# ericyinyzy/VQAttack

Measured on AMD Instinct MI355X. Metric: adversarial_vqa_examples_per_sec, higher is better.
Workload: dtype f32; 1 GPU; vlmo_base VQAttack image PGD (BASELINE configs[1]): batch 64 per GPU, 40 PGD steps, 384x384 images, questions of 6..14 real tokens ([CLS] + n words + [SEP], n ~ U{4..12} seeded) padded to 40 (the all-padding columns are not run through the encoder), eps 0.125 step 0.01 L-inf clip [-1,1], random start, sanity_checks on, black-box scoring + ASR gather; batch_per_gpu=64, pgd_steps=40, image_size=384, text_len=40, substitutable_words=0

## Files before the change

### include/vqattack_hip.h

```cpp
#ifndef VQATTACK_HIP_H
#define VQATTACK_HIP_H

#include <stddef.h>
#include <stdint.h>

#ifdef __cplusplus
extern "C" {
#endif

typedef void* vqa_stream_t;

#define VQA_OK 0
#define VQA_ERR_NULL (-1)
#define VQA_ERR_SHAPE (-2)
#define VQA_ERR_ALIGN (-3)

#define VQA_CLIP 1u
#define VQA_CHECK_RANGE 2u
#define VQA_FLAG_RANGE 1
#define VQA_FLAG_BAD_LABEL 2
#define VQA_FLAG_DEGENERATE 4

int vqa_abi_version(void);
const char* vqa_error_string(int code);
// ... 64 lines not shown
int vqa_neg_cos_max_layers(void);
int vqa_neg_cos_rows_multi(const float* const* a, const float* const* b, float* const* ga, int n_layers,
                           float* partial, const uint8_t* row_mask, long mask_period, long rows0, long rows1, int D,
                           long a_stride0, long a_stride1, long b_stride0, long b_stride1, long g_stride0,
                           long g_stride1, float gscale, float cos_eps, float* loss_out, int accumulate,
                           vqa_stream_t stream);

int vqa_sum_partials(const float* partial, int count, float* dst, int accumulate, float scale,
                     vqa_stream_t stream);

int vqa_ce_max_label_sets(void);
long vqa_ce_scratch_floats(int K, long groups);
int vqa_ce_rows(const float* logits, long row_stride, const int64_t* labels, int K, long rows, int V,
                long ignore_index, long rows_per_group, float* scratch, float* grad, float* row_loss, float gscale,
                float* loss_out, int accumulate, int* flag, unsigned char* row_state, vqa_stream_t stream);

int vqa_gather_rows(const float* src, const int64_t* idx, float* dst, int B, int L, int K, int D,
                    vqa_stream_t stream);

int vqa_cand_dir_sim(const float* word, const float* pos, const float* type, const float* gamma,
                     const float* beta, float ln_eps, const float* e_ori, const float* grad,
                     const int32_t* cand, float* out, int n_cand, int L, int K, int D, vqa_stream_t stream);

int vqa_embed_tokens(const float* word, const float* pos, const float* type, const float* gamma, const float* beta,
                     float ln_eps, const int32_t* triples, int n, float* dst, int D, vqa_stream_t stream);

int vqa_greedy_accept(const int32_t* cand, const int32_t* order, const int32_t* seg, int B, int L,
                      const int64_t* ori_ids, int64_t* cur_ids, int32_t* new_id, int32_t* acc_rank, const float* table,
                      int V, int E, float threshold, vqa_stream_t stream);

int vqa_attn_fwd(const float* q, const float* k, const float* v, const float* bias, float* o, float* lse, float* scores,
                 int B, int H, int Sq, int Sk, const long* strides, const long* bias_strides, float scale,
                 const int* key_hole, int nsplit, float* split_ws, vqa_stream_t stream);
long vqa_attn_scores_floats(int B, int H, int Sq, int Sk);
long vqa_attn_split_ws_floats(int B, int H, int Sq, int Sk, int nsplit);

int vqa_attn_bwd(const float* q, const float* k, const float* v, const float* bias, const float* o, const float* go,
                 const float* lse, const float* scores, float* delta, float* dq, float* dk, float* dv, float* ds_ws, int B,
                 int H, int Sq, int Sk, const long* strides, const long* bias_strides, const long* grad_strides,
                 float scale, int nsplit, float* split_ws, vqa_stream_t stream);
long vqa_attn_bwd_ws_floats(int B, int H, int Sq, int Sk);

int vqa_resize_bicubic_h_u8(const uint8_t* src, int h, int w_in, int c, const int32_t* kk, const int32_t* bounds,
                            int ksize, int w_out, uint8_t* dst, vqa_stream_t stream);
int vqa_resize_bicubic_v_normalize(const uint8_t* src, int h_in, int w, int c, const int32_t* kk,
                                   const int32_t* bounds, int ksize, int h_out, float mean, float stdv, float* dst,
                                   vqa_stream_t stream);

int vqa_ln_fwd(const float* x, const float* r0, const float* r1, const float* rscale, float* x_out,
               const float* gamma0, const float* beta0, const float* gamma1, const float* beta1, float* y0, float* y1,
               float* mean, float* rstd, long rows, int D, long period, long split, float eps, vqa_stream_t stream);
int vqa_ln_bwd(const float* dy0, const float* dy1, const float* x, const float* mean, const float* rstd,
               const float* gamma0, const float* gamma1, const float* g_a, const float* g_inj, const float* rscale,
               float* dx, float* dr0, float* dr1, long rows, int D, long period, long split, vqa_stream_t stream);
int vqa_ln_bwd_post(const float* dy_a, const float* dy_b, const float* g_inj, const float* s, const float* rstd,
                    const float* gamma, float* ds, long rows, int D, vqa_stream_t stream);
int vqa_gelu_fwd(const float* h, float* a, size_t n, vqa_stream_t stream);
int vqa_gelu_bwd(const float* h, const float* da, float* dh, size_t n, vqa_stream_t stream);

size_t vqa_gemm_packed_bytes(int K, int N);
int vqa_gemm_pack_b(const float* w, long ldw, int trans, void* packed, int K, int N, vqa_stream_t stream);
int vqa_gemm_bf16x6(const float* A, long lda, const void* packed, const float* bias, float* C, long ldc, long M, int N,
                    int K, vqa_stream_t stream);

#define VQA_GEMM_TILE_256X128 0
#define VQA_GEMM_TILE_128X256 1
// ... 36 lines not shown
```

### vqattack_amd/_hip.py

```python
import ctypes
import os
import threading

import torch

_HERE = os.path.dirname(os.path.abspath(__file__))
LIB_PATH = os.path.join(_HERE, "lib", "libvqattack_hip.so")
TUNING_LIB_PATH = os.path.join(_HERE, "lib", "libvqattack_hip_tuning.so")

VQA_CLIP = 1
VQA_CHECK_RANGE = 2
VQA_FLAG_RANGE = 1
VQA_FLAG_BAD_LABEL = 2
VQA_FLAG_DEGENERATE = 4
ABI_VERSION = 4

_c_float_p = ctypes.c_void_p
_sz = ctypes.c_size_t
_f = ctypes.c_float
_i = ctypes.c_int
_u = ctypes.c_uint
_l = ctypes.c_long
_p = ctypes.c_void_p

SIGNATURES = {
    "vqa_abi_version": (_i, []),
    "vqa_error_string": (ctypes.c_char_p, [_i]),
    "vqa_linf_init": (_i, [_p, _p, _p, _sz, _f, _f, _f, _u, _p, _p]),
    "vqa_linf_fgm": (_i, [_p, _p, _p, _sz, _f, _f, _f, _u, _p, _p]),
    "vqa_linf_step": (_i, [_p, _p, _p, _p, _sz, _f, _f, _f, _f, _u, _p, _p]),
    "vqa_linf_project": (_i, [_p, _p, _p, _sz, _f, _f, _f, _u, _p]),
    "vqa_clip_eta_linf": (_i, [_p, _p, _sz, _f, _p]),
    "vqa_optimize_linear_linf": (_i, [_p, _p, _sz, _f, _p]),
    "vqa_zero_out_clipped_grads": (_i, [_p, _p, _p, _sz, _f, _f, _p]),
    "vqa_reduce_ws_bytes": (_sz, [_i, _sz]),
    "vqa_sumsq_per_sample": (_i, [_p, _p, _p, _i, _sz, _p, _p]),
    "vqa_absmax_ties_per_sample": (_i, [_p, _p, _p, _i, _sz, _p, _p]),
    "vqa_l2_fgm": (_i, [_p, _p, _p, _p, _i, _sz, _f, _f, _f, _u, _p, _p]),
    "vqa_l2_project": (_i, [_p, _p, _p, _p, _i, _sz, _f, _f, _f, _u, _p]),
    "vqa_l1_fgm": (_i, [_p, _p, _p, _p, _p, _i, _sz, _f, _f, _f, _u, _p, _p]),
    "vqa_scale_per_sample": (_i, [_p, _p, _p, _p, _i, _sz, _f, _i, _p, _p]),
    "vqa_sumabs_per_sample": (_i, [_p, _p, _i, _sz, _p, _p]),
    "vqa_momentum_accumulate": (_i, [_p, _p, _p, _i, _sz, _f, _p]),
    "vqa_linf_momentum_step": (_i, [_p, _p, _p, _p, _p, _p, _i, _sz, _f, _f, _f, _f, _f, _u, _p, _p]),
    "vqa_neg_cos_partials": (_i, []),
    "vqa_neg_cos_rows": (_i, [_p, _p, _p, _p, _p, _l, _l, _l, _i, _l, _l, _l, _l, _l, _l, _f, _f, _p, _i, _p]),
    "vqa_neg_cos_max_layers": (_i, []),
    "vqa_neg_cos_rows_multi": (_i, [_p, _p, _p, _i, _p, _p, _l, _l, _l, _i, _l, _l, _l, _l, _l, _l, _f, _f, _p, _i, _p]),
    "vqa_sum_partials": (_i, [_p, _i, _p, _i, _f, _p]),
    "vqa_ce_max_label_sets": (_i, []),
    "vqa_ce_scratch_floats": (_l, [_i, _l]),
    "vqa_ce_rows": (_i, [_p, _l, _p, _i, _l, _i, _l, _l, _p, _p, _p, _f, _p, _i, _p, _p, _p]),
    "vqa_gather_rows": (_i, [_p, _p, _p, _i, _i, _i, _i, _p]),
    "vqa_cand_dir_sim": (_i, [_p, _p, _p, _p, _p, _f, _p, _p, _p, _p, _i, _i, _i, _i, _p]),
    "vqa_embed_tokens": (_i, [_p, _p, _p, _p, _p, _f, _p, _i, _p, _i, _p]),
    "vqa_greedy_accept": (_i, [_p, _p, _p, _i, _i, _p, _p, _p, _p, _p, _i, _i, _f, _p]),
    "vqa_attn_fwd": (_i, [_p, _p, _p, _p, _p, _p, _p, _i, _i, _i, _i, _p, _p, _f, _p, _i, _p, _p]),
    "vqa_attn_split_ws_floats": (_l, [_i, _i, _i, _i, _i]),
    "vqa_attn_scores_floats": (_l, [_i, _i, _i, _i]),
    "vqa_attn_bwd": (_i, [_p, _p, _p, _p, _p, _p, _p, _p, _p, _p, _p, _p, _p, _i, _i, _i, _i, _p, _p, _p, _f, _i, _p, _p]),
    "vqa_attn_bwd_ws_floats": (_l, [_i, _i, _i, _i]),
    "vqa_ln_fwd": (_i, [_p] * 13 + [_l, _i, _l, _l, _f, _p]),
    "vqa_ln_bwd": (_i, [_p] * 13 + [_l, _i, _l, _l, _p]),
    "vqa_ln_bwd_post": (_i, [_p] * 7 + [_l, _i, _p]),
    "vqa_gelu_fwd": (_i, [_p, _p, _sz, _p]),
    "vqa_gelu_bwd": (_i, [_p, _p, _p, _sz, _p]),
    "vqa_resize_bicubic_h_u8": (_i, [_p, _i, _i, _i, _p, _p, _i, _i, _p, _p]),
    "vqa_resize_bicubic_v_normalize": (_i, [_p, _i, _i, _i, _p, _p, _i, _i, _f, _f, _p, _p]),
    "vqa_gemm_packed_bytes": (_sz, [_i, _i]),
    "vqa_gemm_pack_b": (_i, [_p, _l, _i, _p, _i, _i, _p]),
    "vqa_gemm_bf16x6": (_i, [_p, _l, _p, _p, _p, _l, _l, _i, _i, _p]),
    "vqa_gemm_bf16x6_tile": (_i, [_p, _l, _p, _p, _p, _l, _l, _i, _i, _i, _p]),
    "vqa_gemm_bf16x6_persistent": (_i, [_p, _l, _p, _p, _p, _l, _l, _i, _i, _i, _p]),
    "vqa_gemm_bf16x6_half": (_i, [_p, _l, _p, _p, _p, _l, _l, _i, _i, _p]),
    "vqa_gemm_bf16x6_tail": (_i, [_p, _l, _p, _p, _p, _l, _l, _i, _i, _i, _l, _p]),
    "vqa_gemm_small_ws_bytes": (_sz, [_l, _i, _i]),
    "vqa_gemm_bf16x6_small": (_i, [_p, _l, _p, _p, _p, _l, _l, _i, _i, _i, _p, _p]),
    "vqa_gemm_bf16x6_epi": (_i, [_p, _l, _p, _p, _p, _l, _l, _i, _i, _i, _i, _p, _l, _p]),
    "vqa_gemm_bf16x6_grouped": (_i, [_p, _p, _p, _p, _p, _p, _p, _p, _p, _i, _i, _i, _i, _p]),
    "vqa_gemm_lse_ws_floats": (_l, [_l, _i]),
    "vqa_gemm_bf16x6_lse": (_i, [_p, _l, _p, _p, _l, _i, _i, _i, _p, _l, _p, _p, _p, _p, _i, _p]),
}

_lib = None
_lock = threading.Lock()


class HipExtensionError(RuntimeError):
    pass

# ... 87 lines not shown
```

### vqattack_amd/attention.py

```python
import ctypes

import torch

from . import _hip
from ._hip import check, lib, ptr, stream_for

HEAD_DIM = 64


def _bshd(t, name):
    if not t.is_cuda or t.dtype != torch.float32 or t.dim() != 4 or t.shape[-1] != HEAD_DIM:
        raise _hip.HipExtensionError("{} must be a float32 (B, S, H, 64) HIP tensor, got {} {}".format(
            name, t.dtype, tuple(t.shape)))
    if t.stride(-1) != 1 or any(s % 4 for s in t.stride()[:-1]) or t.data_ptr() % 16:
        t = t.contiguous()
    return t


def _bias_view(bias, b, h, sq, sk):
    if bias is None:
        return None, None
    if bias.dtype != torch.float32 or not bias.is_cuda:
        raise TypeError("bias must be a float32 HIP tensor")
    bias, in_place = _bias_layout(bias, sk)
# ... 40 lines not shown
        pad = torch.zeros(b, 1, 1, sk, device=self.slab.device).masked_fill(masked[:, None, None, :], float("-inf"))
        return self.slab + pad


def _split_hole(bias):
    if isinstance(bias, KeyHoleBias):
        return bias.slab, bias.hole
    return bias, None


_CUS = {}


def loop_split(b, h, sq, sk, device, backward=True):
    import os
    pinned = os.environ.get("VQA_ATTN_SPLIT")
    tiles = ((min(sq, sk) if backward else sk) + 31) // 32
    if pinned:
        return max(1, min(int(pinned), tiles))
    dev = torch.device(device).index or 0
    if dev not in _CUS:
        _CUS[dev] = torch.cuda.get_device_properties(dev).multi_processor_count
    wgs = b * h * ((max(sq, sk) + 127) // 128)
    want = 2 * _CUS[dev]
    if wgs * 2 > want:
        return 1
    return max(1, min(8, tiles // 2, -(-want // wgs)))


def _split_ws(b, h, sq, sk, nsplit, device):
    if nsplit <= 1:
        return None
    return torch.empty(int(lib().vqa_attn_split_ws_floats(b, h, sq, sk, nsplit)), dtype=torch.float32, device=device)


def _forward(q, k, v, bias, bstr, scale, save_scores=False, key_hole=None):
    b, sq, h, _ = q.shape
    sk = k.shape[1]
    nsplit = loop_split(b, h, sq, sk, q.device, backward=False)
    sws = _split_ws(b, h, sq, sk, nsplit, q.device)
    o = torch.empty((b, sq, h, HEAD_DIM), dtype=torch.float32, device=q.device)
    lse = torch.empty((b, h, sq), dtype=torch.float32, device=q.device)
    scores = None
    if save_scores:
        if scores_fit(b, h, sq, sk):
            scores = torch.empty(int(lib().vqa_attn_scores_floats(b, h, sq, sk)), dtype=torch.float32, device=q.device)
        elif key_hole is not None:
            raise _hip.HipExtensionError("a key hole needs the saved-scores backward (the recomputing forms read the "
                                         "padding from the bias): pass KeyHoleBias.dense() at this size")
    strides = _longs([q.stride(0), q.stride(1), q.stride(2), k.stride(0), k.stride(1), k.stride(2),
                      v.stride(0), v.stride(1), v.stride(2), o.stride(0), o.stride(1), o.stride(2)])
    if key_hole is not None and (key_hole.dtype != torch.int32 or tuple(key_hole.shape) != (b, 2) or
                                 not key_hole.is_cuda or not key_hole.is_contiguous()):
        raise TypeError("key_hole must be a contiguous int32 (B, 2) HIP tensor")
    with torch.cuda.device(q.device):
        check(lib().vqa_attn_fwd(ptr(q), ptr(k), ptr(v), ptr(bias), ptr(o), ptr(lse), ptr(scores), b, h, sq, sk, strides,
                                 _longs(bstr) if bstr else None, scale,
                                 None if key_hole is None else ctypes.c_void_p(key_hole.data_ptr()), nsplit, ptr(sws),
                                 stream_for(q)),
              "vqa_attn_fwd")
    return o, lse, scores


def scores_fit(b, h, sq, sk):
    n = int(lib().vqa_attn_scores_floats(b, h, sq, sk))
    return 0 < 4 * n <= SCORES_LIMIT and 0 < 4 * int(lib().vqa_attn_bwd_ws_floats(b, h, sq, sk)) <= DS_WORKSPACE_LIMIT


def _prepare(q, k, v, bias, scale, need_grad=False):
    q, k, v = _bshd(q, "q"), _bshd(k, "k"), _bshd(v, "v")
    b, sq, h, _ = q.shape
    sk = k.shape[1]
    if k.shape != (b, sk, h, HEAD_DIM) or v.shape != k.shape:
        raise ValueError("q / k / v shape mismatch: {} {} {}".format(tuple(q.shape), tuple(k.shape), tuple(v.shape)))
    hole = None
    if isinstance(bias, KeyHoleBias):
        if need_grad and not scores_fit(b, h, sq, sk):
            bias = bias.dense()
        else:
            bias, hole = bias.slab, bias.hole
    bias, bstr = _bias_view(bias, b, h, sq, sk)
    return q, k, v, bias, bstr, HEAD_DIM ** -0.5 if scale is None else float(scale), hole


def attention_forward(q, k, v, bias=None, scale=None):
    q, k, v, bias, bstr, scale, hole = _prepare(q, k, v, bias, scale)
    return _forward(q, k, v, bias, bstr, scale, key_hole=hole)[:2]


DS_WORKSPACE_LIMIT = 8 << 30
SCORES_LIMIT = 6 << 30


# ... 80 lines not shown
```

### vqattack_amd/csrc/attn.hip

```cpp
#include "common.hpp"

namespace vqa {

typedef float f32x4 __attribute__((ext_vector_type(4)));
typedef float f32x16 __attribute__((ext_vector_type(16)));

constexpr int kTile = 32;
constexpr int kKs = 65;

struct AttnDims {
  int B, H, Sq, Sk;
  long q_sb, q_ss, q_sh;
  long k_sb, k_ss, k_sh;
  long v_sb, v_ss, v_sh;
  long o_sb, o_ss, o_sh;
  long bias_sb, bias_sh, bias_sr;
  float scale;
};

#ifdef VQA_TUNING
__device__ int d_attn_ablate = 0;
#define VQA_ABLATE(bit) (d_attn_ablate & (bit))
__device__ unsigned long long* d_attn_stamps = nullptr;
#define VQA_STAMP_DECL unsigned long long stamp_t = 0, stamp_sum[8] = {0, 0, 0, 0, 0, 0, 0, 0}; const bool stamp_on = d_attn_stamps != nullptr;
// ... 298 lines not shown
      store_tile<kKs>(Kbuf[(kt + 1) & 1], tk, 1.0f);
      store_tile_interleaved(Vbuf[(kt + 1) & 1], tv, 1.0f);
    }
    VQA_STAMP(4);
    if (STORE_S && active && !VQA_ABLATE(1)) {
#pragma unroll
      for (int g = 0; g < 4; ++g)
        *reinterpret_cast<f32x4*>(scp + static_cast<long>(kt) * kBlockFloats + 256 * g) =
            f32x4{sraw[4 * g], sraw[4 * g + 1], sraw[4 * g + 2], sraw[4 * g + 3]};
    }
    VQA_STAMP(5);
    __syncthreads();
    VQA_STAMP(6);
  }
  if (active) VQA_STAMP_FLUSH(0, n_tiles - t_lo);
  if (SPLIT) {
    if (qi < d.Sq) {
      l = halves_sum(l);
      const long row = (static_cast<long>(b) * d.H + head) * d.Sq + qi;
      float* wo = sp.ws + (row * nsp + part) * 64;
#pragma unroll
      for (int g = 0; g < 4; ++g) {
        const int dim = 8 * g + 4 * h;
        *reinterpret_cast<f32x4*>(wo + dim) = f32x4{o0[4 * g], o0[4 * g + 1], o0[4 * g + 2], o0[4 * g + 3]};
        *reinterpret_cast<f32x4*>(wo + 32 + dim) = f32x4{o1[4 * g], o1[4 * g + 1], o1[4 * g + 2], o1[4 * g + 3]};
      }
      if (h == 0) {
        float* ml = sp.ws + static_cast<long>(d.B) * d.H * d.Sq * nsp * 64 + (row * nsp + part) * 2;
        ml[0] = m == -INFINITY ? -INFINITY : mc;
        ml[1] = l;
      }
    }
    return;
  }
  if (qi < d.Sq) {
    l = halves_sum(l);
    const float inv = 1.0f / l;
    float* op = o + b * d.o_sb + head * d.o_sh + static_cast<long>(qi) * d.o_ss;
#pragma unroll
    for (int g = 0; g < 4; ++g) {
      const int dim = 8 * g + 4 * h;
      f32x4 a = {o0[4 * g] * inv, o0[4 * g + 1] * inv, o0[4 * g + 2] * inv, o0[4 * g + 3] * inv};
      f32x4 c = {o1[4 * g] * inv, o1[4 * g + 1] * inv, o1[4 * g + 2] * inv, o1[4 * g + 3] * inv};
      *reinterpret_cast<f32x4*>(op + dim) = a;
      *reinterpret_cast<f32x4*>(op + 32 + dim) = c;
    }
    if (h == 0) lse[(static_cast<long>(b) * d.H + head) * d.Sq + qi] = mc * kLn2 + __logf(l);
  }
}


__global__ __launch_bounds__(kBlock) void attn_fwd_combine_kernel(const float* __restrict__ ws, int n,
                                                                  float* __restrict__ o, float* __restrict__ lse,
                                                                  AttnDims d) {
  const long rows = static_cast<long>(d.B) * d.H * d.Sq;
  const long row = static_cast<long>(blockIdx.x) * (kBlock / 16) + threadIdx.x / 16;
  if (row >= rows) return;
  const int c4 = (threadIdx.x & 15) * 4;
  const float* ml = ws + rows * n * 64 + row * n * 2;
  float top = -INFINITY;
  for (int p = 0; p < n; ++p) top = fmaxf(top, ml[2 * p]);
  float l = 0.0f;
  f32x4 acc = {0.0f, 0.0f, 0.0f, 0.0f};
  for (int p = 0; p < n; ++p) {
    const float w = ml[2 * p] == -INFINITY ? 0.0f : __builtin_amdgcn_exp2f(ml[2 * p] - top);
    l += w * ml[2 * p + 1];
// ... 483 lines not shown
static int check_attn(const float* q, const float* k, const float* v, const AttnDims& d) {
  if (!q || !k || !v) return VQA_ERR_NULL;
  if (d.B < 0 || d.H <= 0 || d.Sq <= 0 || d.Sk <= 0 || d.H > 65535 || d.B > 65535) return VQA_ERR_SHAPE;
  const long blocks = ((d.Sq > d.Sk ? d.Sq : d.Sk) + 127L) / 128;
  if (blocks * d.H * d.B > 2147483647L) return VQA_ERR_SHAPE;
  if ((d.q_sb | d.q_ss | d.q_sh | d.k_sb | d.k_ss | d.k_sh | d.v_sb | d.v_ss | d.v_sh | d.o_sb | d.o_ss | d.o_sh) & 3)
    return VQA_ERR_SHAPE;
  if (!aligned16(q) || !aligned16(k) || !aligned16(v)) return VQA_ERR_ALIGN;
  return VQA_OK;
}

long vqa_attn_scores_floats(int B, int H, int Sq, int Sk) {
  if (B < 0 || H <= 0 || Sq <= 0 || Sk <= 0) return 0;
  return static_cast<long>(B) * H * sc_rows(Sq) * sc_pitch(Sk);
}

long vqa_attn_split_ws_floats(int B, int H, int Sq, int Sk, int nsplit) {
  if (B < 0 || H <= 0 || Sq <= 0 || Sk <= 0 || nsplit < 1) return 0;
  if (nsplit == 1) return 0;
  const long rq = static_cast<long>(B) * H * Sq, rk = static_cast<long>(B) * H * Sk;
  const long fwd = split_fwd_floats(rq, nsplit), dkv = 2 * split_sum_floats(rk, nsplit), dq = split_sum_floats(rq, nsplit);
  return fwd > dkv ? (fwd > dq ? fwd : dq) : (dkv > dq ? dkv : dq);
}

static int check_split(int nsplit, const float* split_ws, int tiles, long wgs) {
  if (nsplit < 1) return VQA_ERR_SHAPE;
  if (nsplit == 1) return VQA_OK;
  if (!split_ws) return VQA_ERR_NULL;
  if (!aligned16(split_ws)) return VQA_ERR_ALIGN;
  if (nsplit > tiles || wgs * nsplit > 2147483647L) return VQA_ERR_SHAPE;
  return VQA_OK;
}

int vqa_attn_fwd(const float* q, const float* k, const float* v, const float* bias, float* o, float* lse, float* scores,
                 int B, int H, int Sq, int Sk, const long* strides, const long* bias_strides, float scale,
                 const int* key_hole, int nsplit, float* split_ws, vqa_stream_t stream) {
  clear_stale_error();
  if (!strides || !o || !lse || (bias && !bias_strides)) return VQA_ERR_NULL;
  AttnDims d{B, H, Sq, Sk, strides[0], strides[1], strides[2], strides[3], strides[4], strides[5], strides[6],
             strides[7], strides[8], strides[9], strides[10], strides[11], 0, 0, 0, scale};
  if (bias) {
    d.bias_sb = bias_strides[0];
    d.bias_sh = bias_strides[1];
    d.bias_sr = bias_strides[2];
    if (((d.bias_sb | d.bias_sh | d.bias_sr) & 3) || !aligned16(bias)) return VQA_ERR_ALIGN;
  }
  int rc = check_attn(q, k, v, d);
  if (rc != VQA_OK) return rc;
  if (!aligned16(o) || !aligned16(scores)) return VQA_ERR_ALIGN;
  const long wgs = ((Sq + 127L) / 128) * H * B;
  rc = check_split(nsplit, split_ws, (Sk + kTile - 1) / kTile, wgs);
  if (rc != VQA_OK) return rc;
  if (B == 0) return VQA_OK;
  const dim3 grid(static_cast<unsigned>(wgs * nsplit));
  hipStream_t st = static_cast<hipStream_t>(stream);
  const SplitArgs sp{nsplit, split_ws};
  if (nsplit > 1) {
    if (bias && scores) attn_fwd_kernel<true, true, true><<<grid, kBlock, 0, st>>>(q, k, v, bias, o, lse, scores, d, key_hole, sp);
    else if (bias) attn_fwd_kernel<true, false, true><<<grid, kBlock, 0, st>>>(q, k, v, bias, o, lse, scores, d, key_hole, sp);
    else if (scores) attn_fwd_kernel<false, true, true><<<grid, kBlock, 0, st>>>(q, k, v, bias, o, lse, scores, d, key_hole, sp);
    else attn_fwd_kernel<false, false, true><<<grid, kBlock, 0, st>>>(q, k, v, bias, o, lse, scores, d, key_hole, sp);
    const long rows = static_cast<long>(B) * H * Sq;
    attn_fwd_combine_kernel<<<dim3(static_cast<unsigned>((rows + kBlock / 16 - 1) / (kBlock / 16))), kBlock, 0, st>>>(
        split_ws, nsplit, o, lse, d);
    return launch_status();
  }
  if (bias && scores) attn_fwd_kernel<true, true><<<grid, kBlock, 0, st>>>(q, k, v, bias, o, lse, scores, d, key_hole, sp);
  else if (bias) attn_fwd_kernel<true, false><<<grid, kBlock, 0, st>>>(q, k, v, bias, o, lse, scores, d, key_hole, sp);
  else if (scores) attn_fwd_kernel<false, true><<<grid, kBlock, 0, st>>>(q, k, v, bias, o, lse, scores, d, key_hole, sp);
  else attn_fwd_kernel<false, false><<<grid, kBlock, 0, st>>>(q, k, v, bias, o, lse, scores, d, key_hole, sp);
  return launch_status();
}

long vqa_attn_bwd_ws_floats(int B, int H, int Sq, int Sk) {
  if (B < 0 || H <= 0 || Sq <= 0 || Sk <= 0) return 0;
  return static_cast<long>(B) * H * ds_rows(Sk) * ds_pitch(Sq);
}

int vqa_attn_bwd(const float* q, const float* k, const float* v, const float* bias, const float* o, const float* go,
                 const float* lse, const float* scores, float* delta, float* dq, float* dk, float* dv, float* ds_ws, int B,
                 int H, int Sq, int Sk, const long* strides, const long* bias_strides, const long* grad_strides,
                 float scale, int nsplit, float* split_ws, vqa_stream_t stream) {
  clear_stale_error();
  if (!strides || !grad_strides || !o || !go || !lse || !delta || !dq || !dk || !dv || (bias && !bias_strides))
    return VQA_ERR_NULL;
  AttnDims d{B, H, Sq, Sk, strides[0], strides[1], strides[2], strides[3], strides[4], strides[5], strides[6],
             strides[7], strides[8], strides[9], strides[10], strides[11], 0, 0, 0, scale};
  if (bias) {
    d.bias_sb = bias_strides[0];
    d.bias_sh = bias_strides[1];
    d.bias_sr = bias_strides[2];
    if (((d.bias_sb | d.bias_sh | d.bias_sr) & 3) || !aligned16(bias)) return VQA_ERR_ALIGN;
    if (d.bias_sr < 0 || (static_cast<long>(Sq) + 4) * d.bias_sr + Sk >= 2147483647L) return VQA_ERR_SHAPE;
  }
  const int rc = check_attn(q, k, v, d);
  if (rc != VQA_OK) return rc;
  long any = 0;
  for (int i = 0; i < 12; ++i) any |= grad_strides[i];
  if (any & 3) return VQA_ERR_SHAPE;
  if (!aligned16(o) || !aligned16(go) || !aligned16(dq) || !aligned16(dk) || !aligned16(dv) || !aligned16(ds_ws) ||
      !aligned16(scores))
    return VQA_ERR_ALIGN;
  if (ds_ws && (ds_rows(Sk) * ds_pitch(Sq) >= 2147483647L || sc_rows(Sq) * sc_pitch(Sk) >= 2147483647L))
// ... 74 lines not shown
```

### vqattack_amd/csrc/common.hpp

```cpp
#pragma once
#include <hip/hip_runtime.h>
#include <stdint.h>

#include "../../include/vqattack_hip.h"

namespace vqa {

constexpr int kWave = 64;
constexpr int kBlock = 256;
constexpr int kBlocksPerCu = 8;

#ifdef VQA_TUNING
#define VQA_KNOB static int
#else
#define VQA_KNOB [[maybe_unused]] constexpr int
#endif

__device__ __forceinline__ float sign_torch(float g) {
  return (g > 0.0f ? 1.0f : 0.0f) - (g < 0.0f ? 1.0f : 0.0f);
}

__device__ __forceinline__ float clamp_torch(float v, float lo, float hi) {
  float r = fminf(fmaxf(v, lo), hi);
  return (v != v) ? v : r;
}

__device__ __forceinline__ bool out_of_range(float v, float lo, float hi) {
  return !(v >= lo) || !(v <= hi);
}

struct StepParams {
  float eps_iter, eps, cmin, cmax;
  unsigned mode;
};
struct FgmOp {
  static constexpr int kIn = 2;
  __device__ static float apply(const StepParams& p, float x, float g, float, bool& bad) {
    if (p.mode & VQA_CHECK_RANGE) bad |= out_of_range(x, p.cmin, p.cmax);
    float v = x + p.eps_iter * sign_torch(g);
    return (p.mode & VQA_CLIP) ? clamp_torch(v, p.cmin, p.cmax) : v;
  }
};
struct StepOp {
  static constexpr int kIn = 3;
  __device__ static float apply(const StepParams& p, float x, float g, float x0, bool& bad) {
    if (p.mode & VQA_CHECK_RANGE) bad |= out_of_range(x, p.cmin, p.cmax);
    float a = x + p.eps_iter * sign_torch(g);
    if (p.mode & VQA_CLIP) a = clamp_torch(a, p.cmin, p.cmax);
    float e = clamp_torch(a - x0, -p.eps, p.eps);
    float v = x0 + e;
    return (p.mode & VQA_CLIP) ? clamp_torch(v, p.cmin, p.cmax) : v;
  }
};

template <int CTRL, int ROW_MASK>
__device__ __forceinline__ float dpp_move(float old, float v) {
  return __builtin_bit_cast(float, __builtin_amdgcn_update_dpp(__builtin_bit_cast(int, old), __builtin_bit_cast(int, v),
                                                               CTRL, ROW_MASK, 0xF, false));
}
constexpr int kDppQuadSwap1 = 0xB1;
constexpr int kDppQuadSwap2 = 0x4E;
constexpr int kDppRowHalfMirror = 0x141;
constexpr int kDppRowMirror = 0x140;
constexpr int kDppRowBcast15 = 0x142;
constexpr int kDppRowBcast31 = 0x143;

__device__ __forceinline__ float wave_sum(float v) {
  v += dpp_move<kDppQuadSwap1, 0xF>(0.0f, v);
  v += dpp_move<kDppQuadSwap2, 0xF>(0.0f, v);
  v += dpp_move<kDppRowHalfMirror, 0xF>(0.0f, v);
  v += dpp_move<kDppRowMirror, 0xF>(0.0f, v);
  v += dpp_move<kDppRowBcast15, 0xA>(0.0f, v);
  v += dpp_move<kDppRowBcast31, 0xC>(0.0f, v);
  return __builtin_bit_cast(float, __builtin_amdgcn_readlane(__builtin_bit_cast(int, v), 63));
}

__device__ __forceinline__ float wave_max(float v) {
  v = fmaxf(v, dpp_move<kDppQuadSwap1, 0xF>(v, v));
  v = fmaxf(v, dpp_move<kDppQuadSwap2, 0xF>(v, v));
  v = fmaxf(v, dpp_move<kDppRowHalfMirror, 0xF>(v, v));
  v = fmaxf(v, dpp_move<kDppRowMirror, 0xF>(v, v));
  v = fmaxf(v, dpp_move<kDppRowBcast15, 0xA>(v, v));
  v = fmaxf(v, dpp_move<kDppRowBcast31, 0xC>(v, v));
  return __builtin_bit_cast(float, __builtin_amdgcn_readlane(__builtin_bit_cast(int, v), 63));
}

// ... 62 lines not shown
```

### vqattack_amd/csrc/gemm.hip

```cpp
#include "common.hpp"
#include "gelu.hpp"

namespace vqa {

typedef __bf16 bf16x8 __attribute__((ext_vector_type(8)));
typedef __bf16 bf16x2 __attribute__((ext_vector_type(2)));
typedef float f32x4 __attribute__((ext_vector_type(4)));

constexpr int kGemmBM = 256, kGemmBN = 128, kGemmBK = 32;
constexpr int kGemmThreads = 512;
constexpr int kGemmMT = kGemmBM / 16, kGemmNT = kGemmBN / 16;
constexpr int kTileBytes = 64 * 16;
constexpr int kGemmABytes = kGemmMT * 3 * kTileBytes;
constexpr int kGemmBBytes = kGemmNT * 3 * kTileBytes;
constexpr int kGemmStage = kGemmABytes + kGemmBBytes;
constexpr int kGemmBPieces = kGemmBBytes / 16 / kGemmThreads;
constexpr int kWideLoadPair = 12;

__device__ __forceinline__ void split2(f32x2 a, bf16x2& h0, bf16x2& h1, bf16x2& h2) {
  h0 = __builtin_convertvector(a, bf16x2);
  f32x2 r = a - __builtin_convertvector(h0, f32x2);
  r.x = __builtin_isfinite(r.x) ? r.x : 0.0f;
  r.y = __builtin_isfinite(r.y) ? r.y : 0.0f;
  h1 = __builtin_convertvector(r, bf16x2);
  h2 = __builtin_convertvector(r - __builtin_convertvector(h1, f32x2), bf16x2);
}

__device__ __forceinline__ void split8(const f32x4& lo, const f32x4& hi, bf16x8& p0, bf16x8& p1, bf16x8& p2) {
  bf16x2 a[4], b[4], c[4];
  split2(f32x2{lo.x, lo.y}, a[0], b[0], c[0]);
  split2(f32x2{lo.z, lo.w}, a[1], b[1], c[1]);
  split2(f32x2{hi.x, hi.y}, a[2], b[2], c[2]);
  split2(f32x2{hi.z, hi.w}, a[3], b[3], c[3]);
  p0 = bf16x8{a[0].x, a[0].y, a[1].x, a[1].y, a[2].x, a[2].y, a[3].x, a[3].y};
  p1 = bf16x8{b[0].x, b[0].y, b[1].x, b[1].y, b[2].x, b[2].y, b[3].x, b[3].y};
  p2 = bf16x8{c[0].x, c[0].y, c[1].x, c[1].y, c[2].x, c[2].y, c[3].x, c[3].y};
}

__device__ __forceinline__ void stage_b16(const bf16x8* src, char* lds) {
  __builtin_amdgcn_global_load_lds((const __attribute__((address_space(1))) void*)src,
                                   (__attribute__((address_space(3))) void*)lds, 16, 0, 0);
}
__device__ __forceinline__ void stage_b_wait() { __builtin_amdgcn_s_waitcnt(0x0f70); }

struct GemmArgs {
  const float* A;
  const bf16x8* B;
  const float* bias;
  float* C;
  long lda, ldc, M;
  int N, K;
  int vec;
};

template <bool VEC>
__device__ __forceinline__ f32x4 load4(const float* p) {
  if constexpr (VEC) return *reinterpret_cast<const f32x4*>(p);
  return f32x4{p[0], p[1], p[2], p[3]};
}
template <bool VEC>
__device__ __forceinline__ void store4(float* p, const f32x4& v) {
  if constexpr (VEC) {
    *reinterpret_cast<f32x4*>(p) = v;
  } else {
    p[0] = v.x, p[1] = v.y, p[2] = v.z, p[3] = v.w;
  }
}

template <bool VEC, bool FULL>
__device__ __forceinline__ void gemm_store_rows(const f32x4 (&acc)[4][4], const GemmArgs& g, long row0, int col0, int lane) {
// ... 1401 lines not shown
```

Baseline: 16.28 examples/s.

## Add bf16x6 split-precision MFMA attention forward kernel and make it default

```diff
diff --git a/include/vqattack_hip.h b/include/vqattack_hip.h
--- a/include/vqattack_hip.h
+++ b/include/vqattack_hip.h
@@ -120,6 +120,9 @@
 int vqa_attn_fwd(const float* q, const float* k, const float* v, const float* bias, float* o, float* lse, float* scores,
                  int B, int H, int Sq, int Sk, const long* strides, const long* bias_strides, float scale,
                  const int* key_hole, int nsplit, float* split_ws, vqa_stream_t stream);
+int vqa_attn_fwd_x6(const float* q, const float* k, const float* v, const float* bias, float* o, float* lse,
+                    float* scores, int B, int H, int Sq, int Sk, const long* strides, const long* bias_strides,
+                    float scale, const int* key_hole, int nsplit, float* split_ws, vqa_stream_t stream);
 long vqa_attn_scores_floats(int B, int H, int Sq, int Sk);
 long vqa_attn_split_ws_floats(int B, int H, int Sq, int Sk, int nsplit);
 
diff --git a/vqattack_amd/_hip.py b/vqattack_amd/_hip.py
--- a/vqattack_amd/_hip.py
+++ b/vqattack_amd/_hip.py
@@ -56,6 +56,7 @@
     "vqa_embed_tokens": (_i, [_p, _p, _p, _p, _p, _f, _p, _i, _p, _i, _p]),
     "vqa_greedy_accept": (_i, [_p, _p, _p, _i, _i, _p, _p, _p, _p, _p, _i, _i, _f, _p]),
     "vqa_attn_fwd": (_i, [_p, _p, _p, _p, _p, _p, _p, _i, _i, _i, _i, _p, _p, _f, _p, _i, _p, _p]),
+    "vqa_attn_fwd_x6": (_i, [_p, _p, _p, _p, _p, _p, _p, _i, _i, _i, _i, _p, _p, _f, _p, _i, _p, _p]),
     "vqa_attn_split_ws_floats": (_l, [_i, _i, _i, _i, _i]),
     "vqa_attn_scores_floats": (_l, [_i, _i, _i, _i]),
     "vqa_attn_bwd": (_i, [_p, _p, _p, _p, _p, _p, _p, _p, _p, _p, _p, _p, _p, _i, _i, _i, _i, _p, _p, _p, _f, _i, _p, _p]),
diff --git a/vqattack_amd/attention.py b/vqattack_amd/attention.py
--- a/vqattack_amd/attention.py
+++ b/vqattack_amd/attention.py
@@ -96,6 +96,19 @@
     if nsplit <= 1:
         return None
     return torch.empty(int(lib().vqa_attn_split_ws_floats(b, h, sq, sk, nsplit)), dtype=torch.float32, device=device)
+
+
+FORWARD_DEFAULT = "x6"
+
+
+def forward_grade(nsplit, recomputing_backward=False):
+    import os
+    want = os.environ.get("VQA_ATTN_FWD")
+    if want and want not in ("x6", "f32"):
+        raise ValueError("VQA_ATTN_FWD must be 'x6' or 'f32', got '{}'".format(want))
+    if nsplit != 1 or recomputing_backward:
+        return "f32"
+    return want or FORWARD_DEFAULT
 
 
 def _forward(q, k, v, bias, bstr, scale, save_scores=False, key_hole=None):
@@ -117,12 +130,13 @@
     if key_hole is not None and (key_hole.dtype != torch.int32 or tuple(key_hole.shape) != (b, 2) or
                                  not key_hole.is_cuda or not key_hole.is_contiguous()):
         raise TypeError("key_hole must be a contiguous int32 (B, 2) HIP tensor")
+    entry = "vqa_attn_fwd_x6" if forward_grade(nsplit, save_scores and scores is None) == "x6" else "vqa_attn_fwd"
     with torch.cuda.device(q.device):
-        check(lib().vqa_attn_fwd(ptr(q), ptr(k), ptr(v), ptr(bias), ptr(o), ptr(lse), ptr(scores), b, h, sq, sk, strides,
-                                 _longs(bstr) if bstr else None, scale,
-                                 None if key_hole is None else ctypes.c_void_p(key_hole.data_ptr()), nsplit, ptr(sws),
-                                 stream_for(q)),
-              "vqa_attn_fwd")
+        check(getattr(lib(), entry)(ptr(q), ptr(k), ptr(v), ptr(bias), ptr(o), ptr(lse), ptr(scores), b, h, sq, sk, strides,
+                                    _longs(bstr) if bstr else None, scale,
+                                    None if key_hole is None else ctypes.c_void_p(key_hole.data_ptr()), nsplit, ptr(sws),
+                                    stream_for(q)),
+              entry)
     return o, lse, scores
 
 
diff --git a/vqattack_amd/csrc/attn.hip b/vqattack_amd/csrc/attn.hip
--- a/vqattack_amd/csrc/attn.hip
+++ b/vqattack_amd/csrc/attn.hip
@@ -354,6 +354,222 @@
       }
     }
     return;
+  }
+  if (qi < d.Sq) {
+    l = halves_sum(l);
+    const float inv = 1.0f / l;
+    float* op = o + b * d.o_sb + head * d.o_sh + static_cast<long>(qi) * d.o_ss;
+#pragma unroll
+    for (int g = 0; g < 4; ++g) {
+      const int dim = 8 * g + 4 * h;
+      f32x4 a = {o0[4 * g] * inv, o0[4 * g + 1] * inv, o0[4 * g + 2] * inv, o0[4 * g + 3] * inv};
+      f32x4 c = {o1[4 * g] * inv, o1[4 * g + 1] * inv, o1[4 * g + 2] * inv, o1[4 * g + 3] * inv};
+      *reinterpret_cast<f32x4*>(op + dim) = a;
+      *reinterpret_cast<f32x4*>(op + 32 + dim) = c;
+    }
+    if (h == 0) lse[(static_cast<long>(b) * d.H + head) * d.Sq + qi] = mc * kLn2 + __logf(l);
+  }
+}
+
+constexpr int kX6Plane = 64 * 16;
+constexpr int kX6Tile = 12 * kX6Plane;
+
+__device__ __forceinline__ f32x16 mfma_bf16(const bf16x8& a, const bf16x8& b, f32x16 c) {
+  return __builtin_amdgcn_mfma_f32_32x32x16_bf16(a, b, c, 0, 0, 0);
+}
+
+struct RowCursor {
+  const float* p;
+  const float* last;
+  long step;
+  int last_tile;
+};
+__device__ __forceinline__ RowCursor row_cursor(const float* __restrict__ base, long ss, int n_rows, int lrow, int col) {
+  RowCursor c;
+  c.last_tile = (n_rows - 1) / kTile;
+  int row = c.last_tile * kTile + lrow;
+  row = row < n_rows ? row : n_rows - 1;
+  c.last = base + static_cast<long>(row) * ss + col;
+  c.p = base + static_cast<long>(lrow) * ss + col;
+  c.step = kTile * ss;
+  return c;
+}
+__device__ __forceinline__ const float* row_next(RowCursor& c, int tile) {
+  const float* p = tile == c.last_tile ? c.last : c.p;
+  c.p += c.step;
+  return p;
+}
+
+struct X6Regs {
+  f32x4 k[2], v[2];
+};
+
+template <bool HAS_BIAS, bool STORE_S>
+__global__ __launch_bounds__(kBlock, 2) void attn_fwd_x6_kernel(const float* __restrict__ q, const float* __restrict__ k,
+                                                                const float* __restrict__ v,
+                                                                const float* __restrict__ bias, float* __restrict__ o,
+                                                                float* __restrict__ lse, float* __restrict__ scores,
+                                                                AttnDims d, const int* __restrict__ key_hole) {
+  __shared__ __attribute__((aligned(16))) char Kimg[2][kX6Tile];
+  __shared__ __attribute__((aligned(16))) char Vimg[2][kX6Tile];
+  const int lane = threadIdx.x & (kWave - 1), wave = threadIdx.x / kWave;
+  const int r = lane & 31, h = lane >> 5;
+  const BlockCoord bc = block_coord((d.Sq + 127) / 128, d.B, d.H);
+  const int b = bc.b, head = bc.head;
+  const int q0 = bc.blk * 128 + wave * kTile;
+  const bool active = q0 < d.Sq;
+  const int qi = q0 + r;
+  const int ql = qi < d.Sq ? qi : d.Sq - 1;
+  const float* qp = q + b * d.q_sb + head * d.q_sh + static_cast<long>(ql) * d.q_ss + 32 * h;
+  const float* kb = k + b * d.k_sb + head * d.k_sh;
+  const float* vb = v + b * d.v_sb + head * d.v_sh;
+  const float* bp = HAS_BIAS ? bias + b * d.bias_sb + head * d.bias_sh + static_cast<long>(ql) * d.bias_sr + 4 * h
+                             : nullptr;
+  float* scp = STORE_S ? scores + (static_cast<long>(b) * d.H + head) * sc_rows(d.Sq) * sc_pitch(d.Sk) +
+                             (q0 / kTile) * sc_pitch(d.Sk) * kTile + 4 * lane
+                       : nullptr;
+  bf16x8 qs[3][4];
+#pragma unroll
+  for (int s = 0; s < 4; ++s) {
+    const f32x4 lo = *reinterpret_cast<const f32x4*>(qp + 8 * s) * d.scale;
+    const f32x4 hi = *reinterpret_cast<const f32x4*>(qp + 8 * s + 4) * d.scale;
+    split8<false>(lo, hi, qs[0][s], qs[1][s], qs[2][s]);
+  }
+  f32x16 o0 = {0}, o1 = {0};
+  float m = -INFINITY, mc = 0.0f, l = 0.0f;
+  const int n_tiles = (d.Sk + kTile - 1) / kTile;
+  const int hole_lo = key_hole ? key_hole[2 * b] : 0, hole_hi = key_hole ? key_hole[2 * b + 1] : 0;
+  f32x16 bcur = {0};
+  if (HAS_BIAS && active) bcur = load_bias_tile(bp, 0);
+  const int kc = lane >> 3;
+  RowCursor ck = row_cursor(kb, d.k_ss, d.Sk, 8 * wave + (lane & 7), 8 * kc);
+  const int k_off = ((kc & 3) * 3 * 64 + 32 * (kc >> 2) + 8 * wave + (lane & 7)) * 16;
+  const int kp = threadIdx.x >> 4, dq = threadIdx.x & 15;
+  RowCursor cv0 = row_cursor(vb, d.v_ss, d.Sk, 2 * kp, 4 * dq), cv1 = row_cursor(vb, d.v_ss, d.Sk, 2 * kp + 1, 4 * dq);
+  int v_off[4];
+#pragma unroll
+  for (int e = 0; e < 4; ++e) {
+    const int slot = 32 * ((kp >> 1) & 1) + 4 * (dq & 7) + e;
+    v_off[e] = (((dq >> 3) * 2 + (kp >> 3)) * 3 * 64 + (slot ^ ((slot >> 3) & 3))) * 16 + 4 * (2 * ((kp >> 2) & 1) + (kp & 1));
+  }
+  auto fetch = [&](int tile) {
+    X6Regs t;
+    const float* pk = row_next(ck, tile);
+    t.k[0] = *reinterpret_cast<const f32x4*>(pk);
+    t.k[1] = *reinterpret_cast<const f32x4*>(pk + 4);
+    t.v[0] = *reinterpret_cast<const f32x4*>(row_next(cv0, tile));
+    t.v[1] = *reinterpret_cast<const f32x4*>(row_next(cv1, tile));
+    return t;
+  };
+  auto publish = [&](int buf, const X6Regs& t) {
+    bf16x8 p0, p1, p2;
+    split8<false>(t.k[0], t.k[1], p0, p1, p2);
+    char* kd = Kimg[buf] + k_off;
+    *reinterpret_cast<bf16x8*>(kd) = p0;
+    *reinterpret_cast<bf16x8*>(kd + kX6Plane) = p1;
+    *reinterpret_cast<bf16x8*>(kd + 2 * kX6Plane) = p2;
+#pragma unroll
+    for (int e = 0; e < 4; ++e) {
+      bf16x2 h0, h1, h2;
+      split2<false>(f32x2{t.v[0][e], t.v[1][e]}, h0, h1, h2);
+      char* vd = Vimg[buf] + v_off[e];
+      *reinterpret_cast<bf16x2*>(vd) = h0;
+      *reinterpret_cast<bf16x2*>(vd + kX6Plane) = h1;
+      *reinterpret_cast<bf16x2*>(vd + 2 * kX6Plane) = h2;
+    }
+  };
+  publish(0, fetch(0));
+  __syncthreads();
+  const int v_slot = lane ^ ((lane >> 3) & 3);
+  for (int kt = 0; kt < n_tiles; ++kt) {
+    const int k0 = kt * kTile;
+    const bf16x8* Kf = reinterpret_cast<const bf16x8*>(Kimg[kt & 1]) + lane;
+    const bf16x8* Vf = reinterpret_cast<const bf16x8*>(Vimg[kt & 1]) + v_slot;
+    const bool more = kt + 1 < n_tiles;
+    X6Regs tn;
+    if (more) tn = fetch(kt + 1);
+    f32x16 sraw;
+    if (active) {
+      f32x16 bnext = {0};
+      if (HAS_BIAS && more) bnext = load_bias_tile(bp, k0 + kTile);
+      __builtin_amdgcn_sched_barrier(0);
+      f32x16 st = {0};
+#pragma unroll
+      for (int s = 0; s < 4; ++s) {
+        const bf16x8 kf0 = Kf[(3 * s) * 64], kf1 = Kf[(3 * s + 1) * 64], kf2 = Kf[(3 * s + 2) * 64];
+        st = mfma_bf16(kf2, qs[0][s], st);
+        st = mfma_bf16(kf1, qs[1][s], st);
+        st = mfma_bf16(kf0, qs[2][s], st);
+        st = mfma_bf16(kf1, qs[0][s], st);
+        st = mfma_bf16(kf0, qs[1][s], st);
+        st = mfma_bf16(kf0, qs[0][s], st);
+      }
+      if (HAS_BIAS) st += bcur;
+      if (k0 < hole_hi && k0 + kTile > hole_lo) {
+#pragma unroll
+        for (int i = 0; i < 16; ++i) {
+          const int key = k0 + acc_row(i, h);
+          st[i] = (key >= hole_lo && key < hole_hi) ? -INFINITY : st[i];
+        }
+      }
+      if (STORE_S) sraw = st;
+      if (k0 + kTile > d.Sk) {
+#pragma unroll
+        for (int i = 0; i < 16; ++i) st[i] = k0 + acc_row(i, h) < d.Sk ? st[i] : -INFINITY;
+      }
+      float mx = st[0];
+#pragma unroll
+      for (int i = 1; i < 16; ++i) mx = fmaxf(mx, st[i]);
+      mx = halves_max(mx);
+      const bool grow = mx > m + kLazyMax;
+      if (__builtin_amdgcn_ballot_w64(grow) != 0) {
+        const float m_new = grow ? mx : m;
+        const float mc_new = m_new * kLog2e;
+        const float alpha = m == -INFINITY ? 0.0f : __builtin_amdgcn_exp2f(mc - mc_new);
+        m = m_new;
+        mc = grow ? mc_new : mc;
+        l *= alpha;
+#pragma unroll
+        for (int i = 0; i < 16; ++i) {
+          o0[i] *= alpha;
+          o1[i] *= alpha;
+        }
+      }
+#pragma unroll
+      for (int i = 0; i < 16; ++i) {
+        st[i] = __builtin_amdgcn_exp2f(__builtin_fmaf(st[i], kLog2e, -mc));
+        l += st[i];
+      }
+#pragma unroll
+      for (int s = 0; s < 2; ++s) {
+        bf16x8 p0, p1, p2;
+        split8<false>(f32x4{st[8 * s], st[8 * s + 1], st[8 * s + 2], st[8 * s + 3]},
+                      f32x4{st[8 * s + 4], st[8 * s + 5], st[8 * s + 6], st[8 * s + 7]}, p0, p1, p2);
+        const bf16x8 va0 = Vf[(3 * s) * 64], va1 = Vf[(3 * s + 1) * 64], va2 = Vf[(3 * s + 2) * 64];
+        const bf16x8 vb0 = Vf[(3 * (2 + s)) * 64], vb1 = Vf[(3 * (2 + s) + 1) * 64], vb2 = Vf[(3 * (2 + s) + 2) * 64];
+        o0 = mfma_bf16(va2, p0, o0);
+        o1 = mfma_bf16(vb2, p0, o1);
+        o0 = mfma_bf16(va1, p1, o0);
+        o1 = mfma_bf16(vb1, p1, o1);
+        o0 = mfma_bf16(va0, p2, o0);
+        o1 = mfma_bf16(vb0, p2, o1);
+        o0 = mfma_bf16(va1, p0, o0);
+        o1 = mfma_bf16(vb1, p0, o1);
+        o0 = mfma_bf16(va0, p1, o0);
+        o1 = mfma_bf16(vb0, p1, o1);
+        o0 = mfma_bf16(va0, p0, o0);
+        o1 = mfma_bf16(vb0, p0, o1);
+      }
+      bcur = bnext;
+    }
+    if (more) publish((kt + 1) & 1, tn);
+    if (STORE_S && active) {
+#pragma unroll
+      for (int g = 0; g < 4; ++g)
+        *reinterpret_cast<f32x4*>(scp + static_cast<long>(kt) * kBlockFloats + 256 * g) =
+            f32x4{sraw[4 * g], sraw[4 * g + 1], sraw[4 * g + 2], sraw[4 * g + 3]};
+    }
+    __syncthreads();
   }
   if (qi < d.Sq) {
     l = halves_sum(l);
@@ -903,22 +1119,31 @@
   return VQA_OK;
 }
 
-int vqa_attn_fwd(const float* q, const float* k, const float* v, const float* bias, float* o, float* lse, float* scores,
-                 int B, int H, int Sq, int Sk, const long* strides, const long* bias_strides, float scale,
-                 const int* key_hole, int nsplit, float* split_ws, vqa_stream_t stream) {
-  clear_stale_error();
+static int fwd_dims(const float* q, const float* k, const float* v, const float* bias, const float* o, const float* lse,
+                    const float* scores, int B, int H, int Sq, int Sk, const long* strides, const long* bias_strides,
+                    float scale, AttnDims& d) {
   if (!strides || !o || !lse || (bias && !bias_strides)) return VQA_ERR_NULL;
-  AttnDims d{B, H, Sq, Sk, strides[0], strides[1], strides[2], strides[3], strides[4], strides[5], strides[6],
-             strides[7], strides[8], strides[9], strides[10], strides[11], 0, 0, 0, scale};
+  d = AttnDims{B, H, Sq, Sk, strides[0], strides[1], strides[2], strides[3], strides[4], strides[5], strides[6],
+               strides[7], strides[8], strides[9], strides[10], strides[11], 0, 0, 0, scale};
   if (bias) {
     d.bias_sb = bias_strides[0];
     d.bias_sh = bias_strides[1];
     d.bias_sr = bias_strides[2];
     if (((d.bias_sb | d.bias_sh | d.bias_sr) & 3) || !aligned16(bias)) return VQA_ERR_ALIGN;
   }
-  int rc = check_attn(q, k, v, d);
+  const int rc = check_attn(q, k, v, d);
   if (rc != VQA_OK) return rc;
   if (!aligned16(o) || !aligned16(scores)) return VQA_ERR_ALIGN;
+  return VQA_OK;
+}
+
+int vqa_attn_fwd(const float* q, const float* k, const float* v, const float* bias, float* o, float* lse, float* scores,
+                 int B, int H, int Sq, int Sk, const long* strides, const long* bias_strides, float scale,
+                 const int* key_hole, int nsplit, float* split_ws, vqa_stream_t stream) {
+  clear_stale_error();
+  AttnDims d;
+  int rc = fwd_dims(q, k, v, bias, o, lse, scores, B, H, Sq, Sk, strides, bias_strides, scale, d);
+  if (rc != VQA_OK) return rc;
   const long wgs = ((Sq + 127L) / 128) * H * B;
   rc = check_split(nsplit, split_ws, (Sk + kTile - 1) / kTile, wgs);
   if (rc != VQA_OK) return rc;
@@ -940,6 +1165,25 @@
   else if (bias) attn_fwd_kernel<true, false><<<grid, kBlock, 0, st>>>(q, k, v, bias, o, lse, scores, d, key_hole, sp);
   else if (scores) attn_fwd_kernel<false, true><<<grid, kBlock, 0, st>>>(q, k, v, bias, o, lse, scores, d, key_hole, sp);
   else attn_fwd_kernel<false, false><<<grid, kBlock, 0, st>>>(q, k, v, bias, o, lse, scores, d, key_hole, sp);
+  return launch_status();
+}
+
+int vqa_attn_fwd_x6(const float* q, const float* k, const float* v, const float* bias, float* o, float* lse,
+                    float* scores, int B, int H, int Sq, int Sk, const long* strides, const long* bias_strides,
+                    float scale, const int* key_hole, int nsplit, float* split_ws, vqa_stream_t stream) {
+  clear_stale_error();
+  (void)split_ws;
+  if (nsplit != 1) return VQA_ERR_SHAPE;
+  AttnDims d;
+  const int rc = fwd_dims(q, k, v, bias, o, lse, scores, B, H, Sq, Sk, strides, bias_strides, scale, d);
+  if (rc != VQA_OK) return rc;
+  if (B == 0) return VQA_OK;
+  const dim3 grid(static_cast<unsigned>(((Sq + 127L) / 128) * H * B));
+  hipStream_t st = static_cast<hipStream_t>(stream);
+  if (bias && scores) attn_fwd_x6_kernel<true, true><<<grid, kBlock, 0, st>>>(q, k, v, bias, o, lse, scores, d, key_hole);
+  else if (bias) attn_fwd_x6_kernel<true, false><<<grid, kBlock, 0, st>>>(q, k, v, bias, o, lse, scores, d, key_hole);
+  else if (scores) attn_fwd_x6_kernel<false, true><<<grid, kBlock, 0, st>>>(q, k, v, bias, o, lse, scores, d, key_hole);
+  else attn_fwd_x6_kernel<false, false><<<grid, kBlock, 0, st>>>(q, k, v, bias, o, lse, scores, d, key_hole);
   return launch_status();
 }
 
diff --git a/vqattack_amd/csrc/common.hpp b/vqattack_amd/csrc/common.hpp
--- a/vqattack_amd/csrc/common.hpp
+++ b/vqattack_amd/csrc/common.hpp
@@ -52,6 +52,35 @@
     return (p.mode & VQA_CLIP) ? clamp_torch(v, p.cmin, p.cmax) : v;
   }
 };
+
+typedef __bf16 bf16x8 __attribute__((ext_vector_type(8)));
+typedef __bf16 bf16x2 __attribute__((ext_vector_type(2)));
+typedef float f32x2 __attribute__((ext_vector_type(2)));
+typedef float f32x4 __attribute__((ext_vector_type(4)));
+
+template <bool CHECKED = true>
+__device__ __forceinline__ void split2(f32x2 a, bf16x2& h0, bf16x2& h1, bf16x2& h2) {
+  h0 = __builtin_convertvector(a, bf16x2);
+  f32x2 r = a - __builtin_convertvector(h0, f32x2);
+  if (CHECKED) {
+    r.x = __builtin_isfinite(r.x) ? r.x : 0.0f;
+    r.y = __builtin_isfinite(r.y) ? r.y : 0.0f;
+  }
+  h1 = __builtin_convertvector(r, bf16x2);
+  h2 = __builtin_convertvector(r - __builtin_convertvector(h1, f32x2), bf16x2);
+}
+
+template <bool CHECKED = true>
+__device__ __forceinline__ void split8(const f32x4& lo, const f32x4& hi, bf16x8& p0, bf16x8& p1, bf16x8& p2) {
+  bf16x2 a[4], b[4], c[4];
+  split2<CHECKED>(f32x2{lo.x, lo.y}, a[0], b[0], c[0]);
+  split2<CHECKED>(f32x2{lo.z, lo.w}, a[1], b[1], c[1]);
+  split2<CHECKED>(f32x2{hi.x, hi.y}, a[2], b[2], c[2]);
+  split2<CHECKED>(f32x2{hi.z, hi.w}, a[3], b[3], c[3]);
+  p0 = bf16x8{a[0].x, a[0].y, a[1].x, a[1].y, a[2].x, a[2].y, a[3].x, a[3].y};
+  p1 = bf16x8{b[0].x, b[0].y, b[1].x, b[1].y, b[2].x, b[2].y, b[3].x, b[3].y};
+  p2 = bf16x8{c[0].x, c[0].y, c[1].x, c[1].y, c[2].x, c[2].y, c[3].x, c[3].y};
+}
 
 template <int CTRL, int ROW_MASK>
 __device__ __forceinline__ float dpp_move(float old, float v) {
diff --git a/vqattack_amd/csrc/gemm.hip b/vqattack_amd/csrc/gemm.hip
--- a/vqattack_amd/csrc/gemm.hip
+++ b/vqattack_amd/csrc/gemm.hip
@@ -3,8 +3,6 @@
 
 namespace vqa {
 
-typedef __bf16 bf16x8 __attribute__((ext_vector_type(8)));
-typedef __bf16 bf16x2 __attribute__((ext_vector_type(2)));
 typedef float f32x4 __attribute__((ext_vector_type(4)));
 
 constexpr int kGemmBM = 256, kGemmBN = 128, kGemmBK = 32;
@@ -17,25 +15,6 @@
 constexpr int kGemmBPieces = kGemmBBytes / 16 / kGemmThreads;
 constexpr int kWideLoadPair = 12;
 
-__device__ __forceinline__ void split2(f32x2 a, bf16x2& h0, bf16x2& h1, bf16x2& h2) {
-  h0 = __builtin_convertvector(a, bf16x2);
-  f32x2 r = a - __builtin_convertvector(h0, f32x2);
-  r.x = __builtin_isfinite(r.x) ? r.x : 0.0f;
-  r.y = __builtin_isfinite(r.y) ? r.y : 0.0f;
-  h1 = __builtin_convertvector(r, bf16x2);
-  h2 = __builtin_convertvector(r - __builtin_convertvector(h1, f32x2), bf16x2);
-}
-
-__device__ __forceinline__ void split8(const f32x4& lo, const f32x4& hi, bf16x8& p0, bf16x8& p1, bf16x8& p2) {
-  bf16x2 a[4], b[4], c[4];
-  split2(f32x2{lo.x, lo.y}, a[0], b[0], c[0]);
-  split2(f32x2{lo.z, lo.w}, a[1], b[1], c[1]);
-  split2(f32x2{hi.x, hi.y}, a[2], b[2], c[2]);
-  split2(f32x2{hi.z, hi.w}, a[3], b[3], c[3]);
-  p0 = bf16x8{a[0].x, a[0].y, a[1].x, a[1].y, a[2].x, a[2].y, a[3].x, a[3].y};
-  p1 = bf16x8{b[0].x, b[0].y, b[1].x, b[1].y, b[2].x, b[2].y, b[3].x, b[3].y};
-  p2 = bf16x8{c[0].x, c[0].y, c[1].x, c[1].y, c[2].x, c[2].y, c[3].x, c[3].y};
-}
 
 __device__ __forceinline__ void stage_b16(const bf16x8* src, char* lds) {
   __builtin_amdgcn_global_load_lds((const __attribute__((address_space(1))) void*)src,
```

Result: faster. 16.56 examples/s (median of 6 runs) (+1.7%).
